# OpenVisualCloud/SVT-VP9

Hardware: AMD Instinct MI355X
Metric: hot-path frames/sec (+ Mpixels/sec): block-level DSP path (picture analysis + ME + inter prediction from reconstructed references + DCT/quant/recon + deblock + reference padding), 3840x2160p60 yuv420p enc-mode 8; no mode decision, no entropy coding -- not encoded frames (higher is better)
Workload: dtype u8

## Files before the change

### svt-vp9_amd/csrc/tq_kernel.hip

```cpp
#include <hip/hip_runtime.h>
#include "tq_core.h"

namespace {

template <int N, bool RATE, bool DIST>
__global__ __launch_bounds__(256) __attribute__((amdgpu_waves_per_eu(N == 32 ? (RATE ? 3 : 4) : 1))) void svt_tq_kernel(const uint8_t *__restrict__ src, const uint8_t *__restrict__ pred,
                                                     uint8_t *__restrict__ recon, const svt_tq_block *__restrict__ blocks,
                                                     int n_blocks, const svt_quant_tables *__restrict__ qtabs,
                                                     const int16_t *__restrict__ iscan_all, int16_t *__restrict__ qcoeff,
                                                     int16_t *__restrict__ dqcoeff, uint16_t *__restrict__ eob_out,
                                                     uint64_t *__restrict__ dist_out, tq_rate_args ra, const uint8_t *const *__restrict__ recon_set, tq_dev_count dc) {
    if (dc.p) {
        const int o = dc.p[dc.s];
        n_blocks = dc.p[4 + dc.s];
        blocks += o; eob_out += o;
        if (dc.pos) dc.pos += o;
        if (dist_out) dist_out += 2 * o;
        if constexpr (RATE) ra.bits += o;
    }
    constexpr int NT  = tq_threads<N, RATE>();
    constexpr int BPW = NT / N;
    constexpr int LS  = N + 1;
    __shared__ int32_t tile[BPW][N * LS];
    __shared__ uint32_t s_tc[RATE ? 4 * RATE_SLICE : 1];
    constexpr int SCAN_T = 3 * N * N + 2, SCAN_N = N == 32 ? 3 * N * N : 4 * SCAN_T;
    __shared__ int16_t s_scan[RATE ? SCAN_N : 2];
    if constexpr (RATE) {
        const uint32_t *g = &ra.T->token_costs[txcfg<N>::size][0][0][0][0][0][0];
        for (int j = threadIdx.x; j < 4 * RATE_SLICE; j += NT) s_tc[j] = g[j];
        const uint32_t *gs = (const uint32_t *)(ra.scan + rate_scan_offset(txcfg<N>::size, 0));
        for (int j = threadIdx.x; j < SCAN_N / 2; j += NT) ((uint32_t *)s_scan)[j] = gs[j];
        __syncthreads();
    }
    const int lb  = threadIdx.x / N;
    const int i   = threadIdx.x % N;
    const tq_walk wk = tq_walk_of((n_blocks + BPW - 1) / BPW);
  for (int gj = wk.first; gj < wk.per_xcd; gj += wk.step) {
    const int grp = wk.base + gj;
    if (grp * BPW >= n_blocks) break;
    const int blk = grp * BPW + lb;
    const bool active = blk < n_blocks;
    svt_tq_block k;
    if (dc.pos) {
        const uint32_t pc = dc.pos[active ? blk : 0];
        svt_tq_block_from_pos(pc, txcfg<N>::size, (const svt_tq_pic_geom *)(dc.geom + (size_t)svt_tq_pos_pic(pc) * dc.geom_stride), dc.iscan_off, dc.sb_cols, &k);
    } else if (active) k = blocks[blk];
    else { k = blocks[0]; }
    int32_t *t = tile[lb];
    uint32_t srow[N / 4], prow[N / 4];
    {
        const uint8_t *sp = src + k.src_off + (size_t)i * k.src_stride;
        const uint8_t *pp = pred + k.pred_off + (size_t)i * k.pred_stride;
        constexpr uintptr_t AM = N >= 16 ? 15 : N - 1;
        _Pragma("unroll") for (int q = 0; q < N / 4; q++) { srow[q] = 0u; prow[q] = 0u; }
        if (active) { row_load<N>(sp, ((uintptr_t)sp & AM) == 0, srow); row_load<N>(pp, ((uintptr_t)pp & AM) == 0, prow); }
    }
    int32_t *bits_slot = nullptr;
    if constexpr (RATE) bits_slot = ra.bits + blk;
    tq_block_body<N, RATE, DIST>(k, active, i, t, srow, prow, qtabs, iscan_all, qcoeff, dqcoeff, eob_out + blk, dist_out ? dist_out + 2 * blk : nullptr, bits_slot,
                                 ra.T, s_tc, s_scan, recon_set ? (uint8_t *)recon_set[(k.pad_[0] >> 4) & 7] : recon);
    tq_block_sync();
  }
}


struct scan4_tab { uint8_t scan[16], nb[32]; };
constexpr scan4_tab SCAN4[3] = {
    {{0, 4, 1, 5, 8, 2, 12, 9, 3, 6, 13, 10, 7, 14, 11, 15},
     {0, 0, 0, 0, 0, 0, 1, 4, 4, 4, 1, 1, 8, 8, 5, 8, 2, 2, 2, 5, 9, 12, 6, 9, 3, 6, 10, 13, 7, 10, 11, 14}},
    {{0, 1, 4, 2, 5, 3, 6, 8, 9, 7, 12, 10, 13, 11, 14, 15},
     {0, 0, 0, 0, 0, 0, 1, 1, 4, 4, 2, 2, 5, 5, 4, 4, 8, 8, 6, 6, 8, 8, 9, 9, 12, 12, 10, 10, 13, 13, 14, 14}},
    {{0, 4, 8, 1, 12, 5, 9, 2, 13, 6, 10, 3, 7, 14, 11, 15},
     {0, 0, 0, 0, 4, 4, 0, 0, 8, 8, 1, 1, 5, 5, 1, 1, 9, 9, 2, 2, 6, 6, 2, 2, 3, 3, 10, 10, 7, 7, 11, 11}}};
constexpr uint8_t BAND4[16] = {0, 1, 1, 2, 2, 2, 3, 3, 3, 3, 4, 4, 4, 5, 5, 5};
__host__ __device__ constexpr int scan4_kind(int tx_type) { return tx_type == SVT_ADST_DCT ? 1 : tx_type == SVT_DCT_ADST ? 2 : 0; }

template <int K>
__device__ __forceinline__ int rate_walk4(const int (&tok)[16], const int (&en)[16], const uint32_t *tc, int eob, int ctx0) {
    int sum = (int)tc[ctx0 * 12 + (eob == 0 ? 11 : tok[0])];
    _Pragma("unroll") for (int c = 1; c < 16; c++) {
        if (!__any(c <= eob)) break;
        const int  pt = (1 + en[SCAN4[K].nb[2 * c]] + en[SCAN4[K].nb[2 * c + 1]]) >> 1;
        const bool in = c < eob;
        const int  pz = in && tok[SCAN4[K].scan[c - 1]] == 0, tk = in ? tok[SCAN4[K].scan[c]] : 11;
        const int  v  = (int)tc[((BAND4[c] * 2 + pz) * 6 + pt) * 12 + tk];
        sum += c <= eob ? v : 0;
    }
    return sum;
}

template <int N, bool RATE, bool DIST>
__device__ __forceinline__ void tq_lane_block(const svt_tq_block &k, const int blk, const uint8_t *__restrict__ src, const uint8_t *__restrict__ pred, uint8_t *__restrict__ recon,
                                              const svt_quant_tables *__restrict__ qtabs, const int16_t *__restrict__ iscan_all, int16_t *__restrict__ qcoeff,
                                              int16_t *__restrict__ dqcoeff, uint16_t *__restrict__ eob_out, uint64_t *__restrict__ dist_out, const tq_rate_args &ra,
                                              const uint32_t *s_tc, const int32_t *s_vc, const uint8_t *const *__restrict__ recon_set) {
    constexpr int ND = N / 4;
    const bool col_adst = k.tx_type == SVT_ADST_DCT || k.tx_type == SVT_ADST_ADST;
    const bool row_adst = k.tx_type == SVT_DCT_ADST || k.tx_type == SVT_ADST_ADST;
    const bool dct_dct  = k.tx_type == SVT_DCT_DCT;
    uint32_t   prow[N][ND];
    int32_t    m[N][N];
    {
        uint32_t srow[N][ND];
        _Pragma("unroll") for (int r = 0; r < N; r++) {
            const uint8_t *sp = src + k.src_off + (size_t)r * k.src_stride, *pp = pred + k.pred_off + (size_t)r * k.pred_stride;
            if constexpr (N == 4) { srow[r][0] = *(const uint32_t *)sp; prow[r][0] = *(const uint32_t *)pp; }
            else {
                row_load<N>(sp, ((uintptr_t)sp & 7) == 0, srow[r]);
                row_load<N>(pp, ((uintptr_t)pp & 7) == 0, prow[r]);
            }
        }
        _Pragma("unroll") for (int cc = 0; cc < N; cc++) {
            int32_t v[N], o[N];
            _Pragma("unroll") for (int r = 0; r < N; r++)
                v[r] = ((int)((srow[r][cc >> 2] >> (8 * (cc & 3))) & 0xff) - (int)((prow[r][cc >> 2] >> (8 * (cc & 3))) & 0xff)) * (N == 4 ? 16 : 4);
            if constexpr (N == 4) {
                if (cc == 0 && v[0]) ++v[0];
                if (col_adst) tx_fadst4(v, o); else tx_fdct4(v, o);
            } else {
                if (col_adst) tx_adst8(v, o);
                else if (dct_dct) tx_fdct8(v, o, 0);
                else tx_fdct8(v, o, 1);
            }
            _Pragma("unroll") for (int kk = 0; kk < N; kk++) m[kk][cc] = (int16_t)o[kk];
        }
    }
    svt_quant_tables q;
    {
        const uint32_t *qp = (const uint32_t *)(qtabs + k.qtab);
        uint32_t        qw5[5];
        _Pragma("unroll") for (int j = 0; j < 5; j++) qw5[j] = qp[j];
        q.zbin[0] = (int16_t)qw5[0]; q.zbin[1] = (int16_t)(qw5[0] >> 16); q.round[0] = (int16_t)qw5[1]; q.round[1] = (int16_t)(qw5[1] >> 16);
        q.quant[0] = (int16_t)qw5[2]; q.quant[1] = (int16_t)(qw5[2] >> 16); q.quant_shift[0] = (int16_t)qw5[3]; q.quant_shift[1] = (int16_t)(qw5[3] >> 16);
        q.dequant[0] = (int16_t)qw5[4]; q.dequant[1] = (int16_t)(qw5[4] >> 16);
    }
    int32_t  dq[N][N];
    uint32_t rdist = 0, pdist = 0;
    int      eob = 0;
    int      tok[RATE ? 16 : 1], en[RATE ? 16 : 1], vsum = 0, nnz = 0;
    const uint32_t *ip = (const uint32_t *)(iscan_all + k.iscan_off);
    _Pragma("unroll") for (int i = 0; i < N; i++) {
        int32_t  o[N];
        uint32_t isw[N / 2], qw[N / 2], dqw[N / 2];
        _Pragma("unroll") for (int j = 0; j < N / 2; j++) isw[j] = ip[i * (N / 2) + j];
        if constexpr (N == 4) {
            if (row_adst) tx_fadst4(m[i], o);
            else { tx_fdct4(m[i], o); _Pragma("unroll") for (int kk = 0; kk < N; kk++) o[kk] = (int16_t)o[kk]; }
        } else {
            if (row_adst) tx_adst8(m[i], o);
            else {
                if (dct_dct) tx_fdct8(m[i], o, 0); else tx_fdct8(m[i], o, 1);
                _Pragma("unroll") for (int kk = 0; kk < N; kk++) o[kk] = (int16_t)o[kk];
            }
        }
        _Pragma("unroll") for (int kk = 0; kk < N; kk++) {
            const int cv = N == 4 ? (int16_t)((o[kk] + 1) >> 2) : (int16_t)((o[kk] + (o[kk] < 0)) >> 1);
            const int ac = (i | kk) != 0, sign = cv >> 31, a = (cv ^ sign) - sign;
            int       level = 0, qv = 0, dv = 0;
            if (a >= q.zbin[ac]) {
                const int tmp = clamp16(a + q.round[ac]);
                level = ((((tmp * q.quant[ac]) >> 16) + tmp) * q.quant_shift[ac]) >> 16;
                qv = (int16_t)((level ^ sign) - sign);
                dv = (int16_t)(qv * q.dequant[ac]);
            }
            dq[i][kk] = dv;
            if constexpr (DIST) {
                const int dd = (int16_t)(cv - dv);
                rdist += (uint32_t)(dd * dd);
                pdist += (uint32_t)(cv * cv);
            }
            if (kk & 1) { qw[kk >> 1] |= (uint32_t)(uint16_t)qv << 16; dqw[kk >> 1] |= (uint32_t)(uint16_t)dv << 16; }
            else { qw[kk >> 1] = (uint16_t)qv; dqw[kk >> 1] = (uint16_t)dv; }
            if (level) { const int pos = (int)((isw[kk >> 1] >> (16 * (kk & 1))) & 0xffff) + 1; eob = pos > eob ? pos : eob; }
            if constexpr (RATE) {
                tok[i * N + kk] = 0; en[i * N + kk] = 0;
                if (__any(level != 0)) {
                    const int al = qv < 0 ? -qv : qv;
                    tok[i * N + kk] = token_of(qv);
                    en[i * N + kk]  = energy_of_value(qv);
                    nnz += qv != 0;
                    int vc = s_vc[66 + (al < 67 ? qv : 0)];
                    if (__any(al >= 67)) {
                        const int extra = al >= 67 ? al - 67 : 0;
                        const int c6 = ra.T->cat6_low_cost[extra & 0xff] + ra.T->cat6_high_cost[extra >> 8];
                        vc = al >= 67 ? c6 : vc;
                    }
                    vsum += qv != 0 ? vc : 0;
                }
            }
        }
        int16_t *qo = qcoeff + k.coeff_off + i * N, *dqo = dqcoeff + k.coeff_off + i * N;
        if constexpr (N == 4) { *(uint2 *)qo = make_uint2(qw[0], qw[1]); if (dqcoeff) *(uint2 *)dqo = make_uint2(dqw[0], dqw[1]); }
        else { *(uint4 *)qo = make_uint4(qw[0], qw[1], qw[2], qw[3]); if (dqcoeff) *(uint4 *)dqo = make_uint4(dqw[0], dqw[1], dqw[2], dqw[3]); }
    }
    eob_out[blk] = (uint16_t)eob;
    if constexpr (DIST) if (dist_out) { dist_out[2 * blk] = rdist; dist_out[2 * blk + 1] = pdist; }
    if constexpr (RATE) {
        const int       rinfo = k.pad_[0], ptype = (rinfo >> 2) & 1, inter = (rinfo >> 3) & 1, ctx0 = rinfo & 3;
        const uint32_t *tc = s_tc + (ptype * 2 + inter) * RATE_SLICE;
        const int       kind = scan4_kind(k.tx_type);
        int             bits = 0;
        if (kind == 0) bits = rate_walk4<0>(tok, en, tc, eob, ctx0);
        if (kind == 1) bits = rate_walk4<1>(tok, en, tc, eob, ctx0);
        if (kind == 2) bits = rate_walk4<2>(tok, en, tc, eob, ctx0);
        ra.bits[blk] = bits + vsum + (eob - nnz) * s_vc[66];
    }
    if (!k.do_recon) return;
    constexpr int SH = txcfg<N>::shift;
    uint32_t      rw[N][ND];
    _Pragma("unroll") for (int r = 0; r < N; r++) { _Pragma("unroll") for (int j = 0; j < ND; j++) rw[r][j] = 0; }
    const bool dc_only = dct_dct && (N == 4 ? eob <= 1 : eob == 1);
    if (eob != 0 && !dc_only) {
        int32_t t[N][N];
        _Pragma("unroll") for (int i = 0; i < N; i++) {
            int32_t o[N];
            if constexpr (N == 4) { if (row_adst) tx_iadst4(dq[i], o); else tx_idct4(dq[i], o); }
            else { if (row_adst) tx_adst8(dq[i], o); else tx_idct8(dq[i], o); }
            _Pragma("unroll") for (int kk = 0; kk < N; kk++) t[i][kk] = (int16_t)o[kk];
        }
        _Pragma("unroll") for (int cc = 0; cc < N; cc++) {
            int32_t v[N], o[N];
            _Pragma("unroll") for (int r = 0; r < N; r++) v[r] = t[r][cc];
            if constexpr (N == 4) { if (col_adst) tx_iadst4(v, o); else tx_idct4(v, o); }
            else { if (col_adst) tx_adst8(v, o); else tx_idct8(v, o); }
            _Pragma("unroll") for (int r = 0; r < N; r++) {
                const int res = ((int16_t)o[r] + (1 << (SH - 1))) >> SH;
                rw[r][cc >> 2] |= (uint32_t)clip_add((int)((prow[r][cc >> 2] >> (8 * (cc & 3))) & 0xff), res) << (8 * (cc & 3));
            }
        }
    } else {
        int32_t a1 = 0;
        if (eob != 0) {
            int32_t d = tx_rsw((int16_t)dq[0][0] * TX_C16);
            d = tx_rsw(d * TX_C16);
            a1 = (d + (1 << (SH - 1))) >> SH;
        }
        _Pragma("unroll") for (int r = 0; r < N; r++) {
            _Pragma("unroll") for (int cc = 0; cc < N; cc++)
                rw[r][cc >> 2] |= (uint32_t)clip_add((int)((prow[r][cc >> 2] >> (8 * (cc & 3))) & 0xff), a1) << (8 * (cc & 3));
        }
    }
    uint8_t *const rbase = recon_set ? (uint8_t *)recon_set[(k.pad_[0] >> 4) & 7] : recon;
    if (!rbase) return;
    _Pragma("unroll") for (int r = 0; r < N; r++) {
        uint8_t *d = rbase + k.recon_off + (size_t)r * k.recon_stride;
        if constexpr (N == 4) *(uint32_t *)d = rw[r][0];
        else row_store<N>(d, ((uintptr_t)d & 7) == 0, rw[r]);
    }
}

template <int N, bool RATE, bool DIST>
__global__ __launch_bounds__(256) void svt_tq_lane_kernel(const uint8_t *__restrict__ src, const uint8_t *__restrict__ pred,
                                                          uint8_t *__restrict__ recon, const svt_tq_block *__restrict__ blocks,
                                                          int n_blocks, const svt_quant_tables *__restrict__ qtabs,
                                                          const int16_t *__restrict__ iscan_all, int16_t *__restrict__ qcoeff,
                                                          int16_t *__restrict__ dqcoeff, uint16_t *__restrict__ eob_out,
                                                          uint64_t *__restrict__ dist_out, tq_rate_args ra, const uint8_t *const *__restrict__ recon_set, tq_dev_count dc) {
    if (dc.p) {
        const int o = dc.p[dc.s];
        n_blocks = dc.p[4 + dc.s];
        blocks += o; eob_out += o;
        if (dc.pos) dc.pos += o;
        if (dist_out) dist_out += 2 * o;
        if constexpr (RATE) ra.bits += o;
    }
    static_assert(N == 4 || N == 8, "block-per-lane form: 4x4 and 8x8 only");
    static_assert(!RATE || N == 4, "in-lane rate: 4x4 only");
    __shared__ uint32_t s_tc[RATE ? 4 * RATE_SLICE : 1];
    __shared__ int32_t  s_vc[RATE ? 136 : 1];
    if constexpr (RATE) {
        const uint32_t *g = &ra.T->token_costs[0][0][0][0][0][0][0];
        for (int j = threadIdx.x; j < 4 * RATE_SLICE; j += 256) s_tc[j] = g[j];
        if (threadIdx.x < 133) s_vc[threadIdx.x] = ra.T->value_cost[threadIdx.x];
        __syncthreads();
    }
    const tq_walk wk = tq_walk_of((n_blocks + 255) / 256);
  for (int gj = wk.first; gj < wk.per_xcd; gj += wk.step) {
    const int blk = (wk.base + gj) * 256 + (int)threadIdx.x;
    if (blk >= n_blocks) continue;
    svt_tq_block k;
    if (dc.pos) {
        const uint32_t pc = dc.pos[blk];
        svt_tq_block_from_pos(pc, txcfg<N>::size, (const svt_tq_pic_geom *)(dc.geom + (size_t)svt_tq_pos_pic(pc) * dc.geom_stride), dc.iscan_off, dc.sb_cols, &k);
    } else k = blocks[blk];
    tq_lane_block<N, RATE, DIST>(k, blk, src, pred, recon, qtabs, iscan_all, qcoeff, dqcoeff, eob_out, dist_out, ra, s_tc, s_vc, recon_set);
  }
}

int tq_grid(svt_hip_ctx *ctx, int ngroups, int per_cu) {
    const int per_xcd = (ngroups + 7) / 8, cap = (ctx->cu_count * per_cu + 7) / 8;
    return 8 * (per_xcd < cap ? per_xcd : cap);
}

template <int N, bool RATE, bool DIST = true>
hipError_t launch_tq(svt_hip_ctx *ctx, const uint8_t *src, const uint8_t *pred, uint8_t *recon, const svt_tq_block *blocks, int n,
                     const svt_quant_tables *q, const int16_t *iscan, int16_t *qc, int16_t *dqc, uint16_t *eob, uint64_t *dist, tq_rate_args ra,
                     const uint8_t *const *recon_set, tq_dev_count dc = {nullptr, 0, nullptr, nullptr, 0, nullptr, 0}) {
    if (n <= 0) return hipSuccess;
    if constexpr (N == 4) {
        hipLaunchKernelGGL((svt_tq_lane_kernel<N, RATE, DIST>), dim3(tq_grid(ctx, (n + 255) / 256, 6)), dim3(256), 0, ctx->stream, src, pred, recon, blocks, n, q,
                           iscan, qc, dqc, eob, dist, ra, recon_set, dc);
        return hipGetLastError();
    } else {
        constexpr int NT = tq_threads<N, RATE>(), BPW = NT / N;
        hipLaunchKernelGGL((svt_tq_kernel<N, RATE, DIST>), dim3(tq_grid(ctx, (n + BPW - 1) / BPW, 6)), dim3(NT), 0, ctx->stream, src, pred, recon, blocks, n, q,
                           iscan, qc, dqc, eob, dist, ra, recon_set, dc);
        return hipGetLastError();
    }
}

template <bool RATE>
int32_t tq_launch_all(svt_hip_ctx *ctx, const uint8_t *d_src, const uint8_t *d_pred, uint8_t *d_recon, const svt_tq_block *d_blocks,
                      const int32_t size_count[4], const svt_quant_tables *d_qtabs, const int16_t *d_iscan, int16_t *d_qcoeff,
                      int16_t *d_dqcoeff, uint16_t *d_eob, uint64_t *d_dist, tq_rate_args ra, uint8_t *const *recon_set = nullptr, int n_set = 0) {
    HIP_TRY(hipSetDevice(ctx->device));
    const uint8_t *const *d_set = nullptr;
    if (recon_set) {
        void *h = nullptr, *d = nullptr;
        if (svt_ctx_stage(ctx, 8 * sizeof(void *), &h, &d)) return svt_set_error(SVT_HIP_ERR_NO_RESOURCES, "tq: descriptor buffers");
        for (int i = 0; i < 8; i++) ((uint8_t **)h)[i] = i < n_set ? recon_set[i] : nullptr;
        HIP_TRY(hipMemcpyAsync(d, h, 8 * sizeof(void *), hipMemcpyHostToDevice, ctx->stream));
        d_set = (const uint8_t *const *)d;
    }
    HIP_TRY(hipEventRecord(ctx->ev_start, ctx->stream));
    int        off = 0;
    hipError_t rc = hipSuccess;
    auto at = [&](int o) { tq_rate_args r = ra; if (r.bits) r.bits += o; return r; };
    rc = launch_tq<4, RATE>(ctx, d_src, d_pred, d_recon, d_blocks + off, size_count[0], d_qtabs, d_iscan, d_qcoeff, d_dqcoeff, d_eob + off, d_dist ? d_dist + 2 * off : nullptr, at(off), d_set);
    off += size_count[0];
    if (rc == hipSuccess) rc = launch_tq<8, RATE>(ctx, d_src, d_pred, d_recon, d_blocks + off, size_count[1], d_qtabs, d_iscan, d_qcoeff, d_dqcoeff, d_eob + off, d_dist ? d_dist + 2 * off : nullptr, at(off), d_set);
    off += size_count[1];
    if (rc == hipSuccess) rc = launch_tq<16, RATE>(ctx, d_src, d_pred, d_recon, d_blocks + off, size_count[2], d_qtabs, d_iscan, d_qcoeff, d_dqcoeff, d_eob + off, d_dist ? d_dist + 2 * off : nullptr, at(off), d_set);
    off += size_count[2];
    if (rc == hipSuccess) rc = launch_tq<32, RATE>(ctx, d_src, d_pred, d_recon, d_blocks + off, size_count[3], d_qtabs, d_iscan, d_qcoeff, d_dqcoeff, d_eob + off, d_dist ? d_dist + 2 * off : nullptr, at(off), d_set);
    (void)hipEventRecord(ctx->ev_stop, ctx->stream);
    if (recon_set) svt_ctx_stage_commit(ctx);
    if (rc != hipSuccess) return svt_set_hip_error(rc, __FILE__, __LINE__);
    ctx->timed = 1;
    return SVT_HIP_OK;
}
}

int32_t svt_tq_launch_device_lists(svt_hip_ctx *ctx, const uint8_t *d_src, const uint8_t *d_pred, uint8_t *const *recon_set, int n_set,
                                   const svt_tq_block *d_blocks, const int32_t cap[4], const int32_t *d_off_cnt, const svt_quant_tables *d_qtabs,
                                   const int16_t *d_iscan, int16_t *d_qcoeff, int16_t *d_dqcoeff, uint16_t *d_eob, uint64_t *d_dist,
                                   const uint32_t *d_pos, const void *d_geom, int geom_stride, const uint32_t *d_iscan_off, int sb_cols) {
    HIP_TRY(hipSetDevice(ctx->device));
    void *h = nullptr, *d = nullptr;
    if (svt_ctx_stage(ctx, 8 * sizeof(void *), &h, &d)) return svt_set_error(SVT_HIP_ERR_NO_RESOURCES, "tq: descriptor buffers");
    for (int i = 0; i < 8; i++) ((uint8_t **)h)[i] = i < n_set ? recon_set[i] : nullptr;
    HIP_TRY(hipMemcpyAsync(d, h, 8 * sizeof(void *), hipMemcpyHostToDevice, ctx->stream));
    const uint8_t *const *d_set = (const uint8_t *const *)d;
    const tq_rate_args none = {nullptr, nullptr, nullptr};
    hipError_t rc = hipSuccess;
#define TQ_DEV(N, S, D) launch_tq<N, false, D>(ctx, d_src, d_pred, nullptr, d_blocks, cap[S], d_qtabs, d_iscan, d_qcoeff, d_dqcoeff, d_eob, d_dist, none, d_set, tq_dev_count{d_off_cnt, S, d_pos, (const uint8_t *)d_geom, geom_stride, d_iscan_off, sb_cols})
    if (d_dist) {
        rc = TQ_DEV(4, 0, true);
        if (rc == hipSuccess) rc = TQ_DEV(8, 1, true);
        if (rc == hipSuccess) rc = TQ_DEV(16, 2, true);
        if (rc == hipSuccess) rc = TQ_DEV(32, 3, true);
    } else {
        rc = TQ_DEV(4, 0, false);
        if (rc == hipSuccess) rc = TQ_DEV(8, 1, false);
        if (rc == hipSuccess) rc = TQ_DEV(16, 2, false);
        if (rc == hipSuccess) rc = TQ_DEV(32, 3, false);
    }
#undef TQ_DEV
    svt_ctx_stage_commit(ctx);
    if (rc != hipSuccess) return svt_set_hip_error(rc, __FILE__, __LINE__);
    return SVT_HIP_OK;
}

extern "C" int32_t svt_hip_tq_batch_device(svt_hip_ctx *ctx, const uint8_t *d_src, const uint8_t *d_pred, uint8_t *d_recon,
                                           const svt_tq_block *d_blocks, const int32_t size_count[4],
                                           const svt_quant_tables *d_qtabs, const int16_t *d_iscan, int16_t *d_qcoeff,
                                           int16_t *d_dqcoeff, uint16_t *d_eob) {
    return svt_hip_tq_batch_dist_device(ctx, d_src, d_pred, d_recon, d_blocks, size_count, d_qtabs, d_iscan, d_qcoeff, d_dqcoeff, d_eob,
                                        nullptr);
}

extern "C" int32_t svt_hip_tq_batch_dist_device(svt_hip_ctx *ctx, const uint8_t *d_src, const uint8_t *d_pred, uint8_t *d_recon,
                                                const svt_tq_block *d_blocks, const int32_t size_count[4],
                                                const svt_quant_tables *d_qtabs, const int16_t *d_iscan, int16_t *d_qcoeff,
                                                int16_t *d_dqcoeff, uint16_t *d_eob, uint64_t *d_dist) {
    if (!ctx || !d_src || !d_pred || !d_blocks || !size_count || !d_qtabs || !d_iscan || !d_qcoeff || !d_dqcoeff || !d_eob)
        return svt_set_error(SVT_HIP_ERR_BAD_PARAMETER, "tq: null argument");
    if (((uintptr_t)d_qcoeff | (uintptr_t)d_dqcoeff) & 15) return svt_set_error(SVT_HIP_ERR_BAD_PARAMETER, "tq: coefficient arrays must be 16-byte aligned");
    tq_rate_args none = {nullptr, nullptr, nullptr};
    return tq_launch_all<false>(ctx, d_src, d_pred, d_recon, d_blocks, size_count, d_qtabs, d_iscan, d_qcoeff, d_dqcoeff, d_eob, d_dist, none);
}

extern "C" int32_t svt_hip_tq_rd_batch_device(svt_hip_ctx *ctx, const uint8_t *d_src, const uint8_t *d_pred, uint8_t *d_recon,
                                              const svt_tq_block *d_blocks, const int32_t size_count[4],
                                              const svt_quant_tables *d_qtabs, const int16_t *d_iscan, int16_t *d_qcoeff,
                                              int16_t *d_dqcoeff, uint16_t *d_eob, uint64_t *d_dist,
                                              const svt_rate_tables *d_tables, const int16_t *d_scan, int32_t *d_bits) {
    if (!ctx || !d_src || !d_pred || !d_blocks || !size_count || !d_qtabs || !d_iscan || !d_qcoeff || !d_dqcoeff || !d_eob || !d_tables ||
        !d_scan || !d_bits)
        return svt_set_error(SVT_HIP_ERR_BAD_PARAMETER, "tq_rd: null argument");
    if (((uintptr_t)d_qcoeff | (uintptr_t)d_dqcoeff) & 15) return svt_set_error(SVT_HIP_ERR_BAD_PARAMETER, "tq_rd: coefficient arrays must be 16-byte aligned");
    if ((uintptr_t)d_scan & 3) return svt_set_error(SVT_HIP_ERR_BAD_PARAMETER, "tq_rd: scan array must be 4-byte aligned");
    tq_rate_args ra = {d_tables, d_scan, d_bits};
    return tq_launch_all<true>(ctx, d_src, d_pred, d_recon, d_blocks, size_count, d_qtabs, d_iscan, d_qcoeff, d_dqcoeff, d_eob, d_dist, ra);
}

extern "C" int32_t svt_hip_tq_rd_batch_multi_device(svt_hip_ctx *ctx, const uint8_t *d_src, const uint8_t *d_pred, uint8_t *const *recon_set, int32_t n_set,
                                                    const svt_tq_block *d_blocks, const int32_t size_count[4], const svt_quant_tables *d_qtabs,
                                                    const int16_t *d_iscan, int16_t *d_qcoeff, int16_t *d_dqcoeff, uint16_t *d_eob, uint64_t *d_dist,
                                                    const svt_rate_tables *d_tables, const int16_t *d_scan, int32_t *d_bits) {
    if (!ctx || !d_src || !d_pred || !recon_set || n_set < 1 || n_set > 8 || !d_blocks || !size_count || !d_qtabs || !d_iscan || !d_qcoeff || !d_dqcoeff || !d_eob)
        return svt_set_error(SVT_HIP_ERR_BAD_PARAMETER, "tq_multi: bad argument");
    if (((uintptr_t)d_qcoeff | (uintptr_t)d_dqcoeff) & 15) return svt_set_error(SVT_HIP_ERR_BAD_PARAMETER, "tq_multi: coefficient arrays must be 16-byte aligned");
    if (d_bits) {
        if (!d_tables || !d_scan || ((uintptr_t)d_scan & 3)) return svt_set_error(SVT_HIP_ERR_BAD_PARAMETER, "tq_multi: rate tables / scan array");
        tq_rate_args ra = {d_tables, d_scan, d_bits};
        return tq_launch_all<true>(ctx, d_src, d_pred, nullptr, d_blocks, size_count, d_qtabs, d_iscan, d_qcoeff, d_dqcoeff, d_eob, d_dist, ra, recon_set, n_set);
    }
    tq_rate_args none = {nullptr, nullptr, nullptr};
    return tq_launch_all<false>(ctx, d_src, d_pred, nullptr, d_blocks, size_count, d_qtabs, d_iscan, d_qcoeff, d_dqcoeff, d_eob, d_dist, none, recon_set, n_set);
}

extern "C" int32_t svt_hip_rate_scan4x4_table(int32_t tx_type, int16_t out[48]) {
    if (tx_type < 0 || tx_type > 3 || !out) return svt_set_error(SVT_HIP_ERR_BAD_PARAMETER, "scan4x4: bad argument");
    const scan4_tab &t = SCAN4[scan4_kind(tx_type)];
    for (int i = 0; i < 16; i++) out[i] = t.scan[i];
    for (int i = 0; i < 32; i++) out[16 + i] = t.nb[i];
    return SVT_HIP_OK;
}

extern "C" int32_t svt_hip_tq_batch(svt_hip_ctx *ctx, const uint8_t *src, const uint8_t *pred, uint8_t *recon, size_t plane_bytes,
                                    const svt_tq_block *blocks, int32_t n_blocks, const svt_quant_tables *qtabs, int32_t n_qtabs,
                                    const int16_t *iscan, size_t iscan_count, int16_t *qcoeff, int16_t *dqcoeff,
                                    size_t coeff_count, uint16_t *eob) {
    if (!ctx || !src || !pred || !recon || !blocks || n_blocks < 1 || !qtabs || !iscan || !qcoeff || !dqcoeff || !eob)
        return svt_set_error(SVT_HIP_ERR_BAD_PARAMETER, "tq: null argument");
    int32_t cnt[4] = {0, 0, 0, 0};
    for (int i = 0; i < n_blocks; i++) {
        if (blocks[i].tx_size > 3 || blocks[i].qtab >= n_qtabs) return svt_set_error(SVT_HIP_ERR_BAD_PARAMETER, "tq: bad block");
        if (blocks[i].coeff_off & 7) return svt_set_error(SVT_HIP_ERR_BAD_PARAMETER, "tq: coeff_off must be a multiple of 8 coefficients");
        if (i && blocks[i].tx_size < blocks[i - 1].tx_size) return svt_set_error(SVT_HIP_ERR_BAD_PARAMETER, "tq: blocks not grouped by tx_size");
        if (i && blocks[i].tx_size == blocks[i - 1].tx_size && (blocks[i].do_recon != 0) != (blocks[i - 1].do_recon != 0))
            return svt_set_error(SVT_HIP_ERR_BAD_PARAMETER, "tq: do_recon must be uniform within a tx_size group");
        cnt[blocks[i].tx_size]++;
    }
    HIP_TRY(hipSetDevice(ctx->device));
    uint8_t *ds = (uint8_t *)svt_ctx_slot(ctx, 11, plane_bytes + 64), *dp = (uint8_t *)svt_ctx_slot(ctx, 12, plane_bytes + 64);
    uint8_t *dr = (uint8_t *)svt_ctx_slot(ctx, 13, plane_bytes + 64);
    svt_tq_block *db = (svt_tq_block *)svt_ctx_slot(ctx, 14, sizeof(svt_tq_block) * (size_t)n_blocks);
    svt_quant_tables *dqt = (svt_quant_tables *)svt_ctx_slot(ctx, 15, sizeof(svt_quant_tables) * (size_t)n_qtabs);
    int16_t *dis = (int16_t *)svt_ctx_slot(ctx, 16, sizeof(int16_t) * iscan_count);
    int16_t *dq = (int16_t *)svt_ctx_slot(ctx, 17, sizeof(int16_t) * coeff_count), *ddq = (int16_t *)svt_ctx_slot(ctx, 18, sizeof(int16_t) * coeff_count);
    uint16_t *de = (uint16_t *)svt_ctx_slot(ctx, 19, sizeof(uint16_t) * (size_t)n_blocks);
    if (!ds || !dp || !dr || !db || !dqt || !dis || !dq || !ddq || !de) return svt_set_error(SVT_HIP_ERR_NO_RESOURCES, "tq: device buffers");
    HIP_TRY(hipMemcpyAsync(ds, src, plane_bytes, hipMemcpyHostToDevice, ctx->stream));
    HIP_TRY(hipMemcpyAsync(dp, pred, plane_bytes, hipMemcpyHostToDevice, ctx->stream));
    HIP_TRY(hipMemcpyAsync(dr, recon, plane_bytes, hipMemcpyHostToDevice, ctx->stream));
    HIP_TRY(hipMemcpyAsync(db, blocks, sizeof(svt_tq_block) * (size_t)n_blocks, hipMemcpyHostToDevice, ctx->stream));
    HIP_TRY(hipMemcpyAsync(dqt, qtabs, sizeof(svt_quant_tables) * (size_t)n_qtabs, hipMemcpyHostToDevice, ctx->stream));
    HIP_TRY(hipMemcpyAsync(dis, iscan, sizeof(int16_t) * iscan_count, hipMemcpyHostToDevice, ctx->stream));
    HIP_TRY(hipMemsetAsync(dq, 0, sizeof(int16_t) * coeff_count, ctx->stream));
    HIP_TRY(hipMemsetAsync(ddq, 0, sizeof(int16_t) * coeff_count, ctx->stream));
    int32_t rc = svt_hip_tq_batch_device(ctx, ds, dp, dr, db, cnt, dqt, dis, dq, ddq, de);
    if (rc) return rc;
    HIP_TRY(hipMemcpyAsync(recon, dr, plane_bytes, hipMemcpyDeviceToHost, ctx->stream));
    HIP_TRY(hipMemcpyAsync(qcoeff, dq, sizeof(int16_t) * coeff_count, hipMemcpyDeviceToHost, ctx->stream));
    HIP_TRY(hipMemcpyAsync(dqcoeff, ddq, sizeof(int16_t) * coeff_count, hipMemcpyDeviceToHost, ctx->stream));
    HIP_TRY(hipMemcpyAsync(eob, de, sizeof(uint16_t) * (size_t)n_blocks, hipMemcpyDeviceToHost, ctx->stream));
    HIP_TRY(hipStreamSynchronize(ctx->stream));
    return SVT_HIP_OK;
}
```

Before: 6621.

## Software-pipeline source/prediction row loads in TQ kernels and retune grid sizing

For 4x4 and 8x8 non-rate TQ kernels, the block loop becomes a two-stage software pipeline: the next block's descriptor and source/prediction rows are loaded while the current block is transformed, with an explicit waitcnt barrier before issuing them. Row loading is split out of the per-lane block function so it can be hoisted. The grid-sizing heuristic now takes blocks per two CUs, with per-size defaults for the encoder device-list path (much smaller for 4x4) and an environment override. This trades extra register pressure, since two blocks' rows are live at once, for latency hiding, and changes how many workgroups each size launches.

```diff
diff --git a/svt-vp9_amd/csrc/tq_kernel.hip b/svt-vp9_amd/csrc/tq_kernel.hip
--- a/svt-vp9_amd/csrc/tq_kernel.hip
+++ b/svt-vp9_amd/csrc/tq_kernel.hip
@@ -1,7 +1,12 @@
 #include <hip/hip_runtime.h>
+#include <type_traits>
 #include "tq_core.h"
 
 namespace {
+
+__device__ __forceinline__ void tq_loads_landed() { __builtin_amdgcn_s_waitcnt(0x0F70);  }
+
+template <int N, bool RATE, bool DIST> constexpr bool tq_pipelined() { return N < 16 && !RATE; }
 
 template <int N, bool RATE, bool DIST>
 __global__ __launch_bounds__(256) __attribute__((amdgpu_waves_per_eu(N == 32 ? (RATE ? 3 : 4) : 1))) void svt_tq_kernel(const uint8_t *__restrict__ src, const uint8_t *__restrict__ pred,
@@ -35,32 +40,84 @@
     const int lb  = threadIdx.x / N;
     const int i   = threadIdx.x % N;
     const tq_walk wk = tq_walk_of((n_blocks + BPW - 1) / BPW);
-  for (int gj = wk.first; gj < wk.per_xcd; gj += wk.step) {
-    const int grp = wk.base + gj;
-    if (grp * BPW >= n_blocks) break;
-    const int blk = grp * BPW + lb;
-    const bool active = blk < n_blocks;
-    svt_tq_block k;
-    if (dc.pos) {
-        const uint32_t pc = dc.pos[active ? blk : 0];
-        svt_tq_block_from_pos(pc, txcfg<N>::size, (const svt_tq_pic_geom *)(dc.geom + (size_t)svt_tq_pos_pic(pc) * dc.geom_stride), dc.iscan_off, dc.sb_cols, &k);
-    } else if (active) k = blocks[blk];
-    else { k = blocks[0]; }
-    int32_t *t = tile[lb];
-    uint32_t srow[N / 4], prow[N / 4];
-    {
+    auto in_walk = [&](int gj) { return gj < wk.per_xcd && (wk.base + gj) * BPW < n_blocks; };
+    auto code_of = [&](int gj) { const int blk = (wk.base + gj) * BPW + lb; return dc.pos[blk < n_blocks ? blk : 0]; };
+    auto block_of = [&](auto POS, int gj, uint32_t pc, svt_tq_block &k) {
+        const int blk = (wk.base + gj) * BPW + lb;
+        if constexpr (decltype(POS)::value)
+            svt_tq_block_from_pos(pc, txcfg<N>::size, (const svt_tq_pic_geom *)(dc.geom + (size_t)svt_tq_pos_pic(pc) * dc.geom_stride), dc.iscan_off, dc.sb_cols, &k);
+        else k = blocks[blk < n_blocks ? blk : 0];
+    };
+    auto rows_of = [&](int gj, const svt_tq_block &k, uint32_t (&srow)[N / 4], uint32_t (&prow)[N / 4]) {
+        _Pragma("unroll") for (int q = 0; q < N / 4; q++) { srow[q] = 0u; prow[q] = 0u; }
+        if ((wk.base + gj) * BPW + lb >= n_blocks) return;
         const uint8_t *sp = src + k.src_off + (size_t)i * k.src_stride;
         const uint8_t *pp = pred + k.pred_off + (size_t)i * k.pred_stride;
         constexpr uintptr_t AM = N >= 16 ? 15 : N - 1;
-        _Pragma("unroll") for (int q = 0; q < N / 4; q++) { srow[q] = 0u; prow[q] = 0u; }
-        if (active) { row_load<N>(sp, ((uintptr_t)sp & AM) == 0, srow); row_load<N>(pp, ((uintptr_t)pp & AM) == 0, prow); }
-    }
-    int32_t *bits_slot = nullptr;
-    if constexpr (RATE) bits_slot = ra.bits + blk;
-    tq_block_body<N, RATE, DIST>(k, active, i, t, srow, prow, qtabs, iscan_all, qcoeff, dqcoeff, eob_out + blk, dist_out ? dist_out + 2 * blk : nullptr, bits_slot,
-                                 ra.T, s_tc, s_scan, recon_set ? (uint8_t *)recon_set[(k.pad_[0] >> 4) & 7] : recon);
-    tq_block_sync();
-  }
+        row_load<N>(sp, ((uintptr_t)sp & AM) == 0, srow); row_load<N>(pp, ((uintptr_t)pp & AM) == 0, prow);
+    };
+    auto body_of = [&](int gj, const svt_tq_block &k, const uint32_t (&srow)[N / 4], const uint32_t (&prow)[N / 4]) {
+        const int  blk = (wk.base + gj) * BPW + lb;
+        const bool active = blk < n_blocks;
+        int32_t *bits_slot = nullptr;
+        if constexpr (RATE) bits_slot = ra.bits + blk;
+        tq_block_body<N, RATE, DIST>(k, active, i, tile[lb], srow, prow, qtabs, iscan_all, qcoeff, dqcoeff, eob_out + blk, dist_out ? dist_out + 2 * blk : nullptr, bits_slot,
+                                     ra.T, s_tc, s_scan, recon_set ? (uint8_t *)recon_set[(k.pad_[0] >> 4) & 7] : recon);
+        tq_block_sync();
+    };
+    int gj = wk.first;
+    if constexpr (!tq_pipelined<N, RATE, DIST>()) {
+        for (; gj < wk.per_xcd; gj += wk.step) {
+            const int grp = wk.base + gj;
+            if (grp * BPW >= n_blocks) break;
+            const int blk = grp * BPW + lb;
+            const bool active = blk < n_blocks;
+            svt_tq_block k;
+            if (dc.pos) {
+                const uint32_t pc = dc.pos[active ? blk : 0];
+                svt_tq_block_from_pos(pc, txcfg<N>::size, (const svt_tq_pic_geom *)(dc.geom + (size_t)svt_tq_pos_pic(pc) * dc.geom_stride), dc.iscan_off, dc.sb_cols, &k);
+            } else if (active) k = blocks[blk];
+            else { k = blocks[0]; }
+            int32_t *t = tile[lb];
+            uint32_t srow[N / 4], prow[N / 4];
+            {
+                const uint8_t *sp = src + k.src_off + (size_t)i * k.src_stride;
+                const uint8_t *pp = pred + k.pred_off + (size_t)i * k.pred_stride;
+                constexpr uintptr_t AM = N >= 16 ? 15 : N - 1;
+                _Pragma("unroll") for (int q = 0; q < N / 4; q++) { srow[q] = 0u; prow[q] = 0u; }
+                if (active) { row_load<N>(sp, ((uintptr_t)sp & AM) == 0, srow); row_load<N>(pp, ((uintptr_t)pp & AM) == 0, prow); }
+            }
+            int32_t *bits_slot = nullptr;
+            if constexpr (RATE) bits_slot = ra.bits + blk;
+            tq_block_body<N, RATE, DIST>(k, active, i, t, srow, prow, qtabs, iscan_all, qcoeff, dqcoeff, eob_out + blk, dist_out ? dist_out + 2 * blk : nullptr, bits_slot,
+                                         ra.T, s_tc, s_scan, recon_set ? (uint8_t *)recon_set[(k.pad_[0] >> 4) & 7] : recon);
+            tq_block_sync();
+        }
+    } else {
+        auto walk = [&](auto POS) {
+            constexpr bool P = decltype(POS)::value;
+            bool     have0 = in_walk(gj), have1 = have0 && in_walk(gj + wk.step);
+            uint32_t pc0 = 0u, pc1 = 0u, s0[N / 4], p0[N / 4];
+            if constexpr (P) { if (have0) pc0 = code_of(gj); if (have1) pc1 = code_of(gj + wk.step); }
+            if (have0) { svt_tq_block k; block_of(POS, gj, pc0, k); rows_of(gj, k, s0, p0); }
+            while (have0) {
+                const int  g1 = gj + wk.step, g2 = g1 + wk.step;
+                const bool have2 = have1 && in_walk(g2);
+                uint32_t   pc2 = 0u, s1[N / 4], p1[N / 4];
+                svt_tq_block k, kn;
+                block_of(POS, gj, pc0, k);
+                block_of(POS, have1 ? g1 : gj, have1 ? pc1 : pc0, kn);
+                tq_loads_landed();
+                if (have1) rows_of(g1, kn, s1, p1);
+                else { _Pragma("unroll") for (int q = 0; q < N / 4; q++) { s1[q] = 0u; p1[q] = 0u; } }
+                if constexpr (P) { if (have2) pc2 = code_of(g2); }
+                body_of(gj, k, s0, p0);
+                _Pragma("unroll") for (int q = 0; q < N / 4; q++) { s0[q] = s1[q]; p0[q] = p1[q]; }
+                pc0 = pc1; pc1 = pc2; gj = g1; have0 = have1; have1 = have2;
+            }
+        };
+        if (dc.pos) walk(std::true_type{}); else walk(std::false_type{});
+    }
 }
 
 
@@ -89,8 +146,20 @@
     return sum;
 }
 
+template <int N>
+__device__ __forceinline__ void tq_lane_rows(const svt_tq_block &k, const uint8_t *__restrict__ src, const uint8_t *__restrict__ pred, uint32_t (&srow)[N][N / 4], uint32_t (&prow)[N][N / 4]) {
+    _Pragma("unroll") for (int r = 0; r < N; r++) {
+        const uint8_t *sp = src + k.src_off + (size_t)r * k.src_stride, *pp = pred + k.pred_off + (size_t)r * k.pred_stride;
+        if constexpr (N == 4) { srow[r][0] = *(const uint32_t *)sp; prow[r][0] = *(const uint32_t *)pp; }
+        else {
+            row_load<N>(sp, ((uintptr_t)sp & 7) == 0, srow[r]);
+            row_load<N>(pp, ((uintptr_t)pp & 7) == 0, prow[r]);
+        }
+    }
+}
+
 template <int N, bool RATE, bool DIST>
-__device__ __forceinline__ void tq_lane_block(const svt_tq_block &k, const int blk, const uint8_t *__restrict__ src, const uint8_t *__restrict__ pred, uint8_t *__restrict__ recon,
+__device__ __forceinline__ void tq_lane_block(const svt_tq_block &k, const int blk, const uint32_t (&srow)[N][N / 4], const uint32_t (&prow)[N][N / 4], uint8_t *__restrict__ recon,
                                               const svt_quant_tables *__restrict__ qtabs, const int16_t *__restrict__ iscan_all, int16_t *__restrict__ qcoeff,
                                               int16_t *__restrict__ dqcoeff, uint16_t *__restrict__ eob_out, uint64_t *__restrict__ dist_out, const tq_rate_args &ra,
                                               const uint32_t *s_tc, const int32_t *s_vc, const uint8_t *const *__restrict__ recon_set) {
@@ -98,18 +167,8 @@
     const bool col_adst = k.tx_type == SVT_ADST_DCT || k.tx_type == SVT_ADST_ADST;
     const bool row_adst = k.tx_type == SVT_DCT_ADST || k.tx_type == SVT_ADST_ADST;
     const bool dct_dct  = k.tx_type == SVT_DCT_DCT;
-    uint32_t   prow[N][ND];
     int32_t    m[N][N];
     {
-        uint32_t srow[N][ND];
-        _Pragma("unroll") for (int r = 0; r < N; r++) {
-            const uint8_t *sp = src + k.src_off + (size_t)r * k.src_stride, *pp = pred + k.pred_off + (size_t)r * k.pred_stride;
-            if constexpr (N == 4) { srow[r][0] = *(const uint32_t *)sp; prow[r][0] = *(const uint32_t *)pp; }
-            else {
-                row_load<N>(sp, ((uintptr_t)sp & 7) == 0, srow[r]);
-                row_load<N>(pp, ((uintptr_t)pp & 7) == 0, prow[r]);
-            }
-        }
         _Pragma("unroll") for (int cc = 0; cc < N; cc++) {
             int32_t v[N], o[N];
             _Pragma("unroll") for (int r = 0; r < N; r++)
@@ -275,35 +334,77 @@
         __syncthreads();
     }
     const tq_walk wk = tq_walk_of((n_blocks + 255) / 256);
-  for (int gj = wk.first; gj < wk.per_xcd; gj += wk.step) {
-    const int blk = (wk.base + gj) * 256 + (int)threadIdx.x;
-    if (blk >= n_blocks) continue;
-    svt_tq_block k;
-    if (dc.pos) {
-        const uint32_t pc = dc.pos[blk];
-        svt_tq_block_from_pos(pc, txcfg<N>::size, (const svt_tq_pic_geom *)(dc.geom + (size_t)svt_tq_pos_pic(pc) * dc.geom_stride), dc.iscan_off, dc.sb_cols, &k);
-    } else k = blocks[blk];
-    tq_lane_block<N, RATE, DIST>(k, blk, src, pred, recon, qtabs, iscan_all, qcoeff, dqcoeff, eob_out, dist_out, ra, s_tc, s_vc, recon_set);
-  }
-}
-
-int tq_grid(svt_hip_ctx *ctx, int ngroups, int per_cu) {
-    const int per_xcd = (ngroups + 7) / 8, cap = (ctx->cu_count * per_cu + 7) / 8;
+    auto blk_of = [&](int gj) { return (wk.base + gj) * 256 + (int)threadIdx.x; };
+    auto in_walk = [&](int gj) { return gj < wk.per_xcd && blk_of(gj) < n_blocks; };
+    auto block_of = [&](auto POS, int gj, uint32_t pc, svt_tq_block &k) {
+        if constexpr (decltype(POS)::value) svt_tq_block_from_pos(pc, txcfg<N>::size, (const svt_tq_pic_geom *)(dc.geom + (size_t)svt_tq_pos_pic(pc) * dc.geom_stride), dc.iscan_off, dc.sb_cols, &k);
+        else k = blocks[blk_of(gj)];
+    };
+    if constexpr (!tq_pipelined<N, RATE, DIST>()) {
+      for (int gj = wk.first; gj < wk.per_xcd; gj += wk.step) {
+        const int blk = (wk.base + gj) * 256 + (int)threadIdx.x;
+        if (blk >= n_blocks) continue;
+        svt_tq_block k;
+        if (dc.pos) {
+            const uint32_t pc = dc.pos[blk];
+            svt_tq_block_from_pos(pc, txcfg<N>::size, (const svt_tq_pic_geom *)(dc.geom + (size_t)svt_tq_pos_pic(pc) * dc.geom_stride), dc.iscan_off, dc.sb_cols, &k);
+        } else k = blocks[blk];
+        uint32_t srow[N][N / 4], prow[N][N / 4];
+        tq_lane_rows<N>(k, src, pred, srow, prow);
+        tq_lane_block<N, RATE, DIST>(k, blk, srow, prow, recon, qtabs, iscan_all, qcoeff, dqcoeff, eob_out, dist_out, ra, s_tc, s_vc, recon_set);
+      }
+      return;
+    }
+    auto walk = [&](auto POS) {
+        constexpr bool P = decltype(POS)::value;
+        int      gj = wk.first;
+        bool     have0 = in_walk(gj), have1 = have0 && in_walk(gj + wk.step);
+        uint32_t pc0 = 0u, pc1 = 0u, s0[N][N / 4] = {}, p0[N][N / 4] = {};
+        if constexpr (P) { if (have0) pc0 = dc.pos[blk_of(gj)]; if (have1) pc1 = dc.pos[blk_of(gj + wk.step)]; }
+        if (have0) { svt_tq_block k; block_of(POS, gj, pc0, k); tq_lane_rows<N>(k, src, pred, s0, p0); }
+        while (have0) {
+            const int  g1 = gj + wk.step, g2 = g1 + wk.step;
+            const bool have2 = have1 && in_walk(g2);
+            uint32_t   pc2 = 0u, s1[N][N / 4] = {}, p1[N][N / 4] = {};
+            svt_tq_block k, kn;
+            block_of(POS, gj, pc0, k);
+            block_of(POS, have1 ? g1 : gj, have1 ? pc1 : pc0, kn);
+            tq_loads_landed();
+            if (have1) tq_lane_rows<N>(kn, src, pred, s1, p1);
+            if constexpr (P) { if (have2) pc2 = dc.pos[blk_of(g2)]; }
+            tq_lane_block<N, RATE, DIST>(k, blk_of(gj), s0, p0, recon, qtabs, iscan_all, qcoeff, dqcoeff, eob_out, dist_out, ra, s_tc, s_vc, recon_set);
+            _Pragma("unroll") for (int r = 0; r < N; r++) { _Pragma("unroll") for (int q = 0; q < N / 4; q++) { s0[r][q] = s1[r][q]; p0[r][q] = p1[r][q]; } }
+            pc0 = pc1; pc1 = pc2; gj = g1; have0 = have1; have1 = have2;
+        }
+    };
+    if (dc.pos) walk(std::true_type{}); else walk(std::false_type{});
+}
+
+int tq_grid(svt_hip_ctx *ctx, int ngroups, int per_2cu, int size) {
+    static const struct grid_env { int v[4]; } env = [] {
+        grid_env g = {{0, 0, 0, 0}};
+        if (const char *e = getenv("SVT_HIP_TQ_GRID")) sscanf(e, "%d,%d,%d,%d", &g.v[0], &g.v[1], &g.v[2], &g.v[3]);
+        return g;
+    }();
+    const int per_xcd = (ngroups + 7) / 8, cap = env.v[size] > 0 ? (env.v[size] + 7) / 8 : (ctx->cu_count * per_2cu + 15) / 16;
     return 8 * (per_xcd < cap ? per_xcd : cap);
 }
+
+constexpr int TQ_PER_2CU = 12;
+constexpr int TQ_PER_2CU_ENC[4] = {1, 4, 4, 4};
 
 template <int N, bool RATE, bool DIST = true>
 hipError_t launch_tq(svt_hip_ctx *ctx, const uint8_t *src, const uint8_t *pred, uint8_t *recon, const svt_tq_block *blocks, int n,
                      const svt_quant_tables *q, const int16_t *iscan, int16_t *qc, int16_t *dqc, uint16_t *eob, uint64_t *dist, tq_rate_args ra,
-                     const uint8_t *const *recon_set, tq_dev_count dc = {nullptr, 0, nullptr, nullptr, 0, nullptr, 0}) {
+                     const uint8_t *const *recon_set, tq_dev_count dc = {nullptr, 0, nullptr, nullptr, 0, nullptr, 0}, int per_2cu = TQ_PER_2CU) {
     if (n <= 0) return hipSuccess;
     if constexpr (N == 4) {
-        hipLaunchKernelGGL((svt_tq_lane_kernel<N, RATE, DIST>), dim3(tq_grid(ctx, (n + 255) / 256, 6)), dim3(256), 0, ctx->stream, src, pred, recon, blocks, n, q,
+        hipLaunchKernelGGL((svt_tq_lane_kernel<N, RATE, DIST>), dim3(tq_grid(ctx, (n + 255) / 256, per_2cu, 0)), dim3(256), 0, ctx->stream, src, pred, recon, blocks, n, q,
                            iscan, qc, dqc, eob, dist, ra, recon_set, dc);
         return hipGetLastError();
     } else {
         constexpr int NT = tq_threads<N, RATE>(), BPW = NT / N;
-        hipLaunchKernelGGL((svt_tq_kernel<N, RATE, DIST>), dim3(tq_grid(ctx, (n + BPW - 1) / BPW, 6)), dim3(NT), 0, ctx->stream, src, pred, recon, blocks, n, q,
+        hipLaunchKernelGGL((svt_tq_kernel<N, RATE, DIST>), dim3(tq_grid(ctx, (n + BPW - 1) / BPW, per_2cu, txcfg<N>::size)), dim3(NT), 0, ctx->stream, src, pred, recon, blocks, n, q,
                            iscan, qc, dqc, eob, dist, ra, recon_set, dc);
         return hipGetLastError();
     }
@@ -353,7 +454,7 @@
     const uint8_t *const *d_set = (const uint8_t *const *)d;
     const tq_rate_args none = {nullptr, nullptr, nullptr};
     hipError_t rc = hipSuccess;
-#define TQ_DEV(N, S, D) launch_tq<N, false, D>(ctx, d_src, d_pred, nullptr, d_blocks, cap[S], d_qtabs, d_iscan, d_qcoeff, d_dqcoeff, d_eob, d_dist, none, d_set, tq_dev_count{d_off_cnt, S, d_pos, (const uint8_t *)d_geom, geom_stride, d_iscan_off, sb_cols})
+#define TQ_DEV(N, S, D) launch_tq<N, false, D>(ctx, d_src, d_pred, nullptr, d_blocks, cap[S], d_qtabs, d_iscan, d_qcoeff, d_dqcoeff, d_eob, d_dist, none, d_set, tq_dev_count{d_off_cnt, S, d_pos, (const uint8_t *)d_geom, geom_stride, d_iscan_off, sb_cols}, TQ_PER_2CU_ENC[S])
     if (d_dist) {
         rc = TQ_DEV(4, 0, true);
         if (rc == hipSuccess) rc = TQ_DEV(8, 1, true);
```

After: 6773, median of 6. About the same (+2.3%).
